# fateshelled/sycl_points

Measured on AMD Instinct MI355X. Metric: gicp_correspondences_per_sec, higher is better.
Workload: dtype f32

## Files before the change

sycl_points_amd/_lib.py:

```python
import ctypes as C
import os
import subprocess

_HERE = os.path.dirname(os.path.abspath(__file__))
LIB_PATH = os.environ.get("SP_AMD_LIB") or os.path.join(_HERE, "lib", "libsycl_points_amd.so")
CSRC = os.path.join(_HERE, "csrc")

SP_OK, SP_ERR_INVALID_ARGUMENT, SP_ERR_RUNTIME, SP_ERR_HIP = 0, 1, 2, 3
COMM_ID_BYTES = 128


class SpError(RuntimeError):

    def __init__(self, code, msg):
        super().__init__(f"[sycl_points_amd] error {code}: {msg}")
        self.code = code


class Linearized(C.Structure):
    _fields_ = [("H", C.c_float * 36), ("b", C.c_float * 6), ("error", C.c_float), ("inlier", C.c_uint32),
                ("inlier_lo", C.c_float), ("inlier_hi", C.c_float), ("pad", C.c_float * 2)]


class FactorParams(C.Structure):
# ... 356 lines not shown
    "sp_ogm_extract_visible_points": (_i, [_vp, _vp, _f, _f, _f, _vp, _vp, _vp, _vp, _vp, _sz, C.POINTER(_sz), _vp]),
    "sp_ogm_overlap_ratio": (_i, [_vp, _vp, _sz, _vp, C.POINTER(_f), _vp]),
    "sp_ogm_voxel_probability": (_i, [_vp, _vp, C.POINTER(_f), _vp]),
    "sp_ogm_export": (_i, [_vp, _vp, _vp, _vp, _vp, _vp, _vp, _vp, _vp, _vp, _sz, C.POINTER(_sz), _vp]),
    "sp_pc2_resolve_fields_host": (_i, [C.POINTER(C.c_char_p), C.POINTER(C.c_uint32), C.POINTER(C.c_uint8), _sz, C.c_uint32, _i, _i, _i,
                                        C.POINTER(Pc2Layout)]),
    "sp_pc2_unpack_workspace_bytes": (_sz, [_sz]),
    "sp_pc2_unpack": (_i, [_vp, _sz, _sz, C.POINTER(Pc2Layout), _vp, _vp, _vp, _vp, _vp, _vp, _vp]),
    "sp_pc2_pack_point_step": (C.c_uint32, [_i, _i, _i]),
    "sp_pc2_pack": (_i, [_vp, _vp, _vp, _vp, _sz, C.c_double, _vp, _vp]),
    "sp_enhanced_reflectivity_workspace_bytes": (_sz, [_sz]),
    "sp_enhanced_reflectivity": (_i, [_vp, _vp, _sz, _vp, C.c_uint32, C.c_int32, _i, C.c_int32, _vp, _f, _f, _vp, _vp]),
}


INTERNAL_SIGNATURES = {
    "sp_internal_source_option": (_i, [_vp, _i, _i]),
    "sp_internal_grid_option": (_i, [_vp, _i, _i]),
    "sp_internal_bvh_option": (_i, [_vp, _i, _i]),
    "sp_internal_grid_small_build": (_i, [_i]),
    "sp_internal_align_searched_log": (_vp, [_vp, _vp]),
    "sp_internal_source_tile_floats": (_sz, [_vp]),
    "sp_internal_source_tiles_copy": (_i, [_vp, _vp, _sz, _i, _vp]),
    "sp_internal_radix_sort_workspace_bytes": (_sz, [_sz]),
    "sp_internal_radix_sort_u32": (_i, [_vp, _vp, _vp, _vp, _sz, C.c_uint, _vp, _sz, _vp, _vp]),
    "sp_internal_radix_sort_u32_ex": (_i, [_vp, _vp, _vp, _vp, _sz, C.c_uint, C.c_uint, _i, _vp, _sz, _vp, _vp]),
    "sp_internal_radix_first_pass": (None, [_sz, C.c_uint, _vp]),
    "sp_internal_radix_sort_u64": (_i, [_vp, _vp, _vp, _vp, _sz, C.c_uint, _vp, _sz, _vp, _vp]),
    "sp_internal_exclusive_scan_workspace_bytes": (_sz, [_sz]),
    "sp_internal_exclusive_scan_u32": (_i, [_vp, _vp, _sz, _vp, _vp, _sz, _vp]),
    "sp_internal_atan2f_host": (None, [_vp, _vp, _sz, _vp]),
    "sp_internal_fps": (_i, [_i, _vp, _sz, _sz, C.c_uint32, _vp, _vp, _vp, _vp, _sz, _vp]),
    "sp_internal_eigen3": (_i, [_vp, _sz, _vp, _vp, _vp]),
    "sp_internal_inverse3": (_i, [_vp, _sz, _vp, _vp]),
    "sp_internal_bbox": (_i, [_vp, _sz, C.c_uint, _vp, _vp]),
    "sp_internal_morton_keys": (_i, [_vp, _sz, _vp, _vp, _i, _vp, _vp]),
    "sp_internal_sorted_insert": (_i, [_i, _i, _i, _vp, _vp, _sz, _sz, _vp, _vp, _vp]),
}
VOXEL_BOX_SHARDS, VOXEL_BOX_SHARD_STRIDE = 16, 32
COORD = {"LIDAR": 0, "CAMERA": 1}
FPS_FORM = {"auto": 0, "one_workgroup": 1, "per_sample": 2, "persistent": 3}
INTERNAL_OPTION = {"stage_mask": 0, "reuse": 1, "fast_nn": 2, "self_knn_mode": 3, "persistent": 4, "persistent_from": 5,
                   "bvh_self_heap": 6, "bvh_sort_queries": 7, "grid_sort_queries": 8, "opt_wave_query": 9, "opt_fuse_trials": 10}


def build(force=False):
    srcs = [os.path.join(CSRC, f) for f in os.listdir(CSRC) if f.endswith((".hip", ".h"))]
    srcs.append(os.path.join(_HERE, "..", "include", "sycl_points_amd.h"))
    stale = (not os.path.exists(LIB_PATH)) or any(os.path.getmtime(s) > os.path.getmtime(LIB_PATH) for s in srcs)
    if force or stale:
        subprocess.check_call(["make", "-C", CSRC, "-j8", "-s"])
    return LIB_PATH


_lib = None


def lib():
    global _lib
    if _lib is None:
        if not os.path.exists(LIB_PATH):
            raise ImportError(f"{LIB_PATH} is missing: run `python -c 'import __graft_entry__ as g; g.build()'` "
                              "(there is no CPU fallback for the HIP path)")
        import torch

        L = C.CDLL(LIB_PATH)
        for name, (res, args) in list(SIGNATURES.items()) + list(INTERNAL_SIGNATURES.items()):
            fn = getattr(L, name)
            fn.restype = res
            fn.argtypes = args
        if L.sp_abi_version() != 7:
            raise ImportError("libsycl_points_amd.so ABI version mismatch")
        _lib = L
    return _lib


def check(code):
    if code != SP_OK:
        raise SpError(code, lib().sp_last_error().decode())
```

sycl_points_amd/csrc/grid_device.h:

```cpp
#pragma once
#include "sp_common.h"
#include "sp_math.h"

struct sp_grid {
    size_t n = 0;
    float h = 1.0f, inv_h = 1.0f, eps = 0.0f;
    float org[3] = {0, 0, 0};
    int dims[3] = {1, 1, 1};
    size_t ncells = 1;
    float4* d_pts = nullptr;
    uint32_t* d_start = nullptr;
    mutable uint32_t* d_unit_off = nullptr;
    mutable uint32_t n_units = 0;
    mutable bool units_ready = false;
    hipStream_t build_stream = nullptr;
    hipEvent_t built_ev = nullptr;
    mutable uint32_t max_cell = 0;
    mutable bool max_cell_known = false;
    int self_knn_mode = 0;
    int sort_queries = 1;
    mutable sp::StreamSet streams;
};

namespace sp {

inline void grid_use(const sp_grid* g, hipStream_t st) {
    if (g->built_ev != nullptr && st != g->build_stream) (void)hipStreamWaitEvent(st, g->built_ev, 0);
    g->streams.note(st);
}

int grid_search_own_points(const sp_grid* grid, size_t k, int32_t* idx_out, float* d2_out, hipStream_t st, float bound2 = FLT_MAX);

struct GridDesc {
    float inv_h, h, eps;
    float ox, oy, oz;
    int nx, ny, nz;
    unsigned n;
};

inline GridDesc grid_desc(const sp_grid* gr) {
    return GridDesc{gr->inv_h, gr->h, gr->eps, gr->org[0], gr->org[1], gr->org[2], gr->dims[0], gr->dims[1],
                    gr->dims[2], (unsigned)gr->n};
}

__device__ __forceinline__ int cell_coord(float v, float o, float inv_h, int dim) {
    const float t = floorf((v - o) * inv_h);
    return (int)fminf(fmaxf(t, 0.0f), (float)(dim - 1));
}

__device__ __forceinline__ float gap2(float v, float lo, float hi, float eps) {
    const float g = fmaxf(fmaxf(lo - v, v - hi) - eps, 0.0f);
    return g * g;
}

__device__ __forceinline__ void load4_dist2(const float4* __restrict__ pts, unsigned i, unsigned e, float qx, float qy, float qz,
                                            float4 (&p)[4], float (&d)[4]) {
#pragma unroll
    for (int j = 0; j < 4; ++j) p[j] = pts[j ? min(i + j, e - 1) : i];
#pragma unroll
    for (int j = 0; j < 4; ++j) d[j] = dist2(qx, qy, qz, p[j].x, p[j].y, p[j].z);
}

template <class Bound, class Scan>
__device__ __forceinline__ void grid_ring_walk(const unsigned* __restrict__ start, const GridDesc& g, float qx, float qy,
                                               float qz, int r_start, bool proven_before, Bound&& bound2, Scan&& scan) {
// ... 36 lines not shown
                }
            }
        }
        if (covered(r)) break;
    }
}

struct Nearest {
    float d2;
    int idx;
    unsigned pos;
    float x, y, z;
};

__device__ __forceinline__ Nearest grid_nn1(const float4* __restrict__ pts, const unsigned* __restrict__ start,
                                            const GridDesc& g, float qx, float qy, float qz,
                                            const Nearest* seed = nullptr, int r_start = 0) {
    Nearest best;
    best.d2 = FLT_MAX; best.idx = -1; best.pos = 0; best.x = best.y = best.z = 0.0f;
    if (!(isfinite(qx) && isfinite(qy) && isfinite(qz)) || g.n == 0) return best;
    if (seed) best = *seed;
    const int cx = cell_coord(qx, g.ox, g.inv_h, g.nx), cy = cell_coord(qy, g.oy, g.inv_h, g.ny),
              cz = cell_coord(qz, g.oz, g.inv_h, g.nz);
    const int rmax = max(max(g.nx, g.ny), g.nz);
    auto consider = [&](const float4 p, unsigned pos) {
        const float d = dist2(qx, qy, qz, p.x, p.y, p.z);
        const int pi = __float_as_int(p.w);
        if (d < best.d2 || (d == best.d2 && pi < best.idx)) {
            best.d2 = d; best.idx = pi; best.pos = pos; best.x = p.x; best.y = p.y; best.z = p.z;
        }
    };
    for (int r = r_start; r <= rmax; ++r) {
        const int z0 = max(cz - r, 0), z1 = min(cz + r, g.nz - 1);
        const int y0 = max(cy - r, 0), y1 = min(cy + r, g.ny - 1);
        const int x0 = max(cx - r, 0), x1 = min(cx + r, g.nx - 1);
        for (int z = z0; z <= z1; ++z) {
            const float dz2 = gap2(qz, g.oz + z * g.h, g.oz + (z + 1) * g.h, g.eps);
            if (dz2 > best.d2) continue;
            for (int y = y0; y <= y1; ++y) {
                const float dyz2 = dz2 + gap2(qy, g.oy + y * g.h, g.oy + (y + 1) * g.h, g.eps);
                if (dyz2 > best.d2) continue;
                const bool shell_row = (r == 0) || (z == cz - r) || (z == cz + r) || (y == cy - r) || (y == cy + r);
                const unsigned row = ((unsigned)z * g.ny + y) * g.nx;
                const int nseg = shell_row ? 1 : 2;
                for (int sgi = 0; sgi < nseg; ++sgi) {
                    int xa, xb;
                    if (shell_row) { xa = x0; xb = x1; }
// ... 14 lines not shown
                    }
                }
            }
        }
        float cov = FLT_MAX;
        if (cx - r > 0) cov = fminf(cov, qx - (g.ox + (cx - r) * g.h));
        if (cx + r < g.nx - 1) cov = fminf(cov, (g.ox + (cx + r + 1) * g.h) - qx);
        if (cy - r > 0) cov = fminf(cov, qy - (g.oy + (cy - r) * g.h));
        if (cy + r < g.ny - 1) cov = fminf(cov, (g.oy + (cy + r + 1) * g.h) - qy);
        if (cz - r > 0) cov = fminf(cov, qz - (g.oz + (cz - r) * g.h));
        if (cz + r < g.nz - 1) cov = fminf(cov, (g.oz + (cz + r + 1) * g.h) - qz);
        if (cov == FLT_MAX) break;
        cov = fmaxf(cov - g.eps, 0.0f);
        if (best.d2 < cov * cov) break;
    }
    return best;
}

struct FastFlat {
    unsigned o0, o1, o2, o3;
    unsigned c1, c2, c3, total;
};

__device__ __forceinline__ void fast_extents(const unsigned* __restrict__ start, const GridDesc& g, float qx, float qy,
                                             float qz, unsigned (&s)[4], unsigned (&e)[4], float& cov_cells) {
    const float fx = (qx - g.ox) * g.inv_h, fy = (qy - g.oy) * g.inv_h, fz = (qz - g.oz) * g.inv_h;
    const float cxf = fminf(fmaxf(floorf(fx), 0.0f), (float)(g.nx - 1));
    const float cyf = fminf(fmaxf(floorf(fy), 0.0f), (float)(g.ny - 1));
    const float czf = fminf(fmaxf(floorf(fz), 0.0f), (float)(g.nz - 1));
    const float tx = fx - cxf, ty = fy - cyf, tz = fz - czf;
    const bool lx = tx < 0.5f, ly = ty < 0.5f, lz = tz < 0.5f;
    const int cx = (int)cxf, cy = (int)cyf, cz = (int)czf;
    const int xa = max(cx - (lx ? 1 : 0), 0), xb = min(cx + (lx ? 0 : 1), g.nx - 1);
    const int ya = max(cy - (ly ? 1 : 0), 0), yb = min(cy + (ly ? 0 : 1), g.ny - 1);
    const int za = max(cz - (lz ? 1 : 0), 0), zb = min(cz + (lz ? 0 : 1), g.nz - 1);
    cov_cells = fminf(fminf(lx ? 1.0f - tx : tx, ly ? 1.0f - ty : ty), lz ? 1.0f - tz : tz);
    const unsigned r00 = ((unsigned)za * g.ny + ya) * g.nx + xa;
    const unsigned dy = yb != ya ? (unsigned)g.nx : 0u, dz = zb != za ? (unsigned)g.ny * g.nx : 0u;
    const unsigned w = (unsigned)(xb - xa) + 1u;
    const unsigned r01 = r00 + dy, r10 = r00 + dz, r11 = r10 + dy;
    struct Three { unsigned a, b, c; };
    const Three v0 = *reinterpret_cast<const Three*>(start + r00), v1 = *reinterpret_cast<const Three*>(start + r01),
                v2 = *reinterpret_cast<const Three*>(start + r10), v3 = *reinterpret_cast<const Three*>(start + r11);
    const bool two = w == 2u;
    s[0] = v0.a; e[0] = two ? v0.c : v0.b;
    s[1] = v1.a; e[1] = two ? v1.c : v1.b;
    s[2] = v2.a; e[2] = two ? v2.c : v2.b;
    s[3] = v3.a; e[3] = two ? v3.c : v3.b;
    if (dy == 0u) { e[1] = s[1]; e[3] = s[3]; }
    if (dz == 0u) { e[2] = s[2]; e[3] = s[3]; }
}

__device__ __forceinline__ FastFlat fast_flatten(const unsigned (&s)[4], const unsigned (&e)[4], bool usable) {
    FastFlat f;
    const unsigned n0 = e[0] - s[0], n1 = e[1] - s[1], n2 = e[2] - s[2], n3 = e[3] - s[3];
    f.c1 = n0; f.c2 = n0 + n1; f.c3 = f.c2 + n2;
    f.o0 = s[0]; f.o1 = s[1] - f.c1; f.o2 = s[2] - f.c2; f.o3 = s[3] - f.c3;
    f.total = usable ? f.c3 + n3 : 0u;
    return f;
}
__device__ __forceinline__ unsigned fast_pos(const FastFlat& f, unsigned jj) {
    return jj + (jj < f.c1 ? f.o0 : (jj < f.c2 ? f.o1 : (jj < f.c3 ? f.o2 : f.o3)));
}

template <int B>
__device__ __forceinline__ void fast_load(const float4* __restrict__ pts, const FastFlat& f, unsigned base,
                                          float4 (&cand)[B]) {
#pragma unroll
    for (int j = 0; j < B; ++j) cand[j] = pts[fast_pos(f, min(base + j, f.total - 1))];
}
__device__ __forceinline__ unsigned long long nn_key(float d2, int idx) {
    return ((unsigned long long)__float_as_uint(d2) << 32) | (unsigned)idx;
}
template <int B>
__device__ __forceinline__ void fast_eval(const FastFlat& f, unsigned base, const float4 (&cand)[B], float qx, float qy,
                                          float qz, unsigned long long& best_key, unsigned& bj) {
#pragma unroll
    for (int j = 0; j < B; ++j) {
        const float d = dist2(qx, qy, qz, cand[j].x, cand[j].y, cand[j].z);
        unsigned long long key = nn_key(d, __float_as_int(cand[j].w));
        key = (base + j < f.total) ? key : ~0ull;
        const bool better = key < best_key;
        best_key = better ? key : best_key;
        bj = better ? base + j : bj;
    }
}

__device__ __forceinline__ bool grid_nn1_fast(const float4* __restrict__ pts, const unsigned* __restrict__ start,
                                              const GridDesc& g, float qx, float qy, float qz, Nearest& best,
                                              float bound2 = FLT_MAX, const Nearest* seed = nullptr) {
    best.d2 = bound2; best.idx = -1; best.pos = 0; best.x = best.y = best.z = 0.0f;
    const bool usable = isfinite(qx) && isfinite(qy) && isfinite(qz) && g.n != 0;
    if (!usable) return true;
    if (seed) best = *seed;
    unsigned s[4], e[4];
    float cov_cells;
    fast_extents(start, g, qx, qy, qz, s, e, cov_cells);
    const FastFlat f = fast_flatten(s, e, true);
    const unsigned long long none = nn_key(best.d2, best.idx);
    unsigned long long key = none;
    unsigned bj = 0;
#ifndef SP_FAST_B
#define SP_FAST_B 12
#endif
    for (unsigned base = 0; base < f.total; base += SP_FAST_B) {
        float4 cand[SP_FAST_B];
        fast_load<SP_FAST_B>(pts, f, base, cand);
        fast_eval<SP_FAST_B>(f, base, cand, qx, qy, qz, key, bj);
    }
    if (key != none) {
        best.pos = fast_pos(f, bj);
        const float4 w = pts[best.pos];
        best.x = w.x; best.y = w.y; best.z = w.z;
        best.idx = __float_as_int(w.w);
        best.d2 = __uint_as_float((unsigned)(key >> 32));
    }
    const float cov = fmaxf(cov_cells * g.h - g.eps, 0.0f);
    return best.d2 < cov * cov;
}

// ... 237 lines not shown
    second2 = ub;
    if (winner != kNone && runner_up != kNone) second2 = fminf(ub, __uint_as_float((unsigned)(runner_up >> 32)));
    if (m < key_in) {
        const int wl = __ffsll((long long)__ballot(k1 == m)) - 1;
        const unsigned wpos = (unsigned)__builtin_amdgcn_readlane((int)bpos, wl);
        const float4 w = pts[wpos];
        best.d2 = __uint_as_float((unsigned)(m >> 32));
        best.idx = __float_as_int(w.w);
        best.pos = wpos;
        best.x = w.x; best.y = w.y; best.z = w.z;
    }
}

__device__ __forceinline__ void grid_nn1_later_stages(const float4* __restrict__ pts, const unsigned* __restrict__ start,
                                                      const GridDesc& g, float qx, float qy, float qz, Nearest& best) {
    if (grid_nn1_block4(pts, start, g, qx, qy, qz, best)) return;
    if (best.d2 < FLT_MAX && grid_nn1_ball(pts, start, g, qx, qy, qz, best)) return;
    const Nearest seed = best;
    best = grid_nn1(pts, start, g, qx, qy, qz, &seed, 2);
}

__device__ __forceinline__ Nearest grid_nn1_auto(const float4* __restrict__ pts, const unsigned* __restrict__ start,
                                                 const GridDesc& g, float qx, float qy, float qz, float bound2 = FLT_MAX,
                                                 const Nearest* seed = nullptr) {
    Nearest best;
    if (!grid_nn1_fast(pts, start, g, qx, qy, qz, best, bound2, seed)) grid_nn1_later_stages(pts, start, g, qx, qy, qz, best);
    return best;
}

}
```

sycl_points_amd/csrc/registration.hip:

```cpp
#include <algorithm>
#include <mutex>

#include "registration_device.h"
#include "sp_cov_normal.h"

namespace sp {
namespace {


struct PointTerm {
    float H[6][6];
    float b[6];
    float sq;
    float residual_norm;
    float genz_weight;
};

__device__ __forceinline__ void se3_jacobian(const Rigid& T, float px, float py, float pz, float J[3][6]) {
#pragma unroll
    for (int i = 0; i < 3; ++i) {
        const float r0 = T.R[i][0], r1 = T.R[i][1], r2 = T.R[i][2];
        J[i][0] = chain3(r0, 0.0f, r1, pz, r2, -py);
        J[i][1] = chain3(r0, -pz, r1, 0.0f, r2, px);
        J[i][2] = chain3(r0, py, r1, -px, r2, 0.0f);
// ... 636 lines not shown
            after_loads();
            if (threadIdx.x < kFanRow) red[1][threadIdx.x] = rv;
        }
        __syncthreads();
        if (threadIdx.x < kAcc - 1) red[0][threadIdx.x] = red[1][threadIdx.x];
        else if (threadIdx.x == kAcc - 1)
            red[0][kAcc - 1] = __uint_as_float((unsigned)red[1][kAcc] * 4096u + (unsigned)red[1][kAcc - 1]);
        else if (threadIdx.x == kAcc) red[0][kAcc] = red[1][kAcc + 1];
        __syncthreads();
        return true;
    }
}
__device__ __forceinline__ void align_store_late_state(const AlignArgs& A) {
    if (threadIdx.x < kStateWords) {
        unsigned w = A.has_prev ? reinterpret_cast<const unsigned*>(A.state_in)[threadIdx.x] : 0u;
        if (!A.has_prev && threadIdx.x < 16) w = __float_as_uint(A.T_init[threadIdx.x]);
        if (threadIdx.x == kStateFlagWord) w = 1u;
        if (threadIdx.x == kStateFlagWord + 3) w = 1u;
        reinterpret_cast<unsigned*>(A.state_out)[threadIdx.x] = w;
    }
}

template <bool SHARDED>
__device__ __forceinline__ bool align_prologue(const AlignArgs& A, float* sT, unsigned* sflag) {
    __shared__ float red[kFinalThreads / 32][kPartial];
    __shared__ sp_linearized slin;
    __shared__ float sdelta[8];
    __shared__ LdltScratch ldlt_ws;
    if (A.first) {
        state_store(state_load(false, nullptr, A.T_init), sT, sflag);
        if (!SHARDED && blockIdx.x == 0 && A.searched_log && threadIdx.x >= 64 && threadIdx.x < 64 + kSearchedLog)
            A.searched_log[threadIdx.x - 64] = 0u;
        __syncthreads();
        return true;
    }
    const unsigned sv = state_load(A.has_prev, A.state_in, A.T_init);
    const unsigned nrows = (SHARDED && A.mode == ALIGN_ROWS) ? (unsigned)kAlignMaxBlocks : gridDim.x;
    const bool arrived = align_totals<SHARDED>(A, A.prev_rows, nrows, red, [=] { state_store(sv, sT, sflag); }, sflag);
    if (!arrived) {
        if (blockIdx.x == 0) align_store_late_state(A);
        return false;
    }
    auto zero_row = [&] {
        if (SHARDED && A.mode == ALIGN_FANIN && blockIdx.x == 0 && threadIdx.x >= 64 && threadIdx.x < 64 + kFanRow)
            A.fan_row_out[threadIdx.x - 64] = 0.0f;
    };
    if (sflag[0]) {
        if (blockIdx.x == 0 && threadIdx.x < kStateWords)
            reinterpret_cast<unsigned*>(A.state_out)[threadIdx.x] = reinterpret_cast<const unsigned*>(A.state_in)[threadIdx.x];
        zero_row();
        return false;
    }
    if (threadIdx.x == 0)
        finish_iteration(red[0], sT, A.lambda, A.crit_rot, A.crit_trans, sflag[1], &slin, sdelta, &ldlt_ws, blockIdx.x == 0, A.state_out,
                         A.searched_log,
                         A.k, A.lin_out);
    __syncthreads();
    if (sdelta[6] > 0.5f) {
        zero_row();
        return false;
    }
    return true;
}

template <int LOSS, bool FAST_NN, bool P2D = false, bool SHARDED = false>
__global__ __launch_bounds__(kAlignBlock) void gicp_align_kernel(FusedParams P, AlignArgs A,
                                                                 float* __restrict__ partials) {
    __shared__ float sT[16];
    __shared__ unsigned sflag[2];
    if (!align_prologue<SHARDED>(A, sT, sflag)) return;
    const Rigid T = uniform_pose(sT);
    float acc[kAcc - 1];
    unsigned cnt = 0, searched = 0;
    const unsigned stride = gridDim.x * kAlignBlock;
#pragma unroll
    for (int e = 0; e < kAcc - 1; ++e) acc[e] = 0.0f;
    const unsigned tile = xcd_tile();
    for (unsigned i = tile * kAlignBlock + threadIdx.x; i < P.n; i += stride)
        fused_point<LOSS, FAST_NN, P2D, kSeedSearches, kNegCert>(P, T, i, acc, cnt, searched);
    if constexpr (!SHARDED) {
        block_reduce_store<kAcc - 1, kAlignBlock>(acc, cnt, partials + (size_t)blockIdx.x * kPartial, false, searched);
    } else if (A.mode == ALIGN_ROWS) {
        block_reduce_store<kAcc - 1, kAlignBlock>(acc, cnt, partials + (size_t)blockIdx.x * kPartial, true, searched);
    } else {
        block_reduce_store<kAcc - 1, kAlignBlock, true>(acc, cnt, partials + (size_t)blockIdx.x * kPartial, false, searched);
        align_tail(A, partials);
    }
}

struct PersistArgs {
    AlignWs ws;
    unsigned* tickets;
    const float* T_init;
    float lambda, crit_rot, crit_trans;
    sp_linearized* lin_out;
    float* T_out;
    float* delta_out8;
    uint32_t* iterations_out;
    int max_iterations;
    int k_begin;
    int cache_valid_later;
    unsigned long long budget;
// ... 899 lines not shown
    return SP_OK;
}

extern "C" int sp_gicp_source_set_wave_per_point(sp_gicp_source* s, int mode) {
    if (!s || mode < 0 || mode > 2) return SP_ERR_INVALID_ARGUMENT;
    s->opt_wave_query = mode;
    return SP_OK;
}

extern "C" const uint32_t* sp_internal_align_searched_log(void* workspace, size_t* n_entries_out) {
    if (n_entries_out) *n_entries_out = sp::kSearchedLog;
    return workspace ? sp::align_ws(workspace).searched_log : nullptr;
}
extern "C" size_t sp_internal_source_tile_floats(const sp_gicp_source* s) {
    return s ? sp::src_tile_words(s->n_max ? s->n_max : 1) : 0;
}
extern "C" int sp_internal_source_tiles_copy(sp_gicp_source* s, float* device_buffer, size_t n_floats, int to_source, void* stream) {
    if (!s || !device_buffer || n_floats != sp_internal_source_tile_floats(s)) return SP_ERR_INVALID_ARGUMENT;
    const hipError_t e = hipMemcpyAsync(to_source ? s->tiles : device_buffer, to_source ? device_buffer : s->tiles,
                                        n_floats * sizeof(float), hipMemcpyDeviceToDevice, sp::as_stream(stream));
    if (e != hipSuccess) { sp_set_error(hipGetErrorString(e)); return SP_ERR_HIP; }
    return SP_OK;
}
extern "C" int sp_internal_source_option(sp_gicp_source* s, int option, int value) {
    if (!s) return SP_ERR_INVALID_ARGUMENT;
    switch (option) {
        case SP_INTERNAL_FUSED_STAGE_MASK: s->opt_stage_mask = value; return SP_OK;
        case SP_INTERNAL_FUSED_REUSE: s->opt_reuse = value; s->cache_valid = false; return SP_OK;
        case SP_INTERNAL_FUSED_FAST_NN: s->opt_fast_nn = value; return SP_OK;
        case SP_INTERNAL_FUSED_PERSISTENT: s->opt_persistent = value; return SP_OK;
        case SP_INTERNAL_FUSED_PERSISTENT_FROM: s->opt_persistent_from = value < 0 ? 0 : value; return SP_OK;
        case SP_INTERNAL_OPT_WAVE_QUERY: s->opt_wave_query = value; return SP_OK;
        case SP_INTERNAL_OPT_FUSE_TRIALS: s->opt_fuse_trials = value; return SP_OK;
    }
    return SP_ERR_INVALID_ARGUMENT;
}
```

sycl_points_amd/csrc/registration_device.h:

```cpp
#ifndef SP_REGISTRATION_DEVICE_H
#define SP_REGISTRATION_DEVICE_H

#include "grid_device.h"
#include "radix_sort.h"
#include "sp_linearize.h"
#include "sp_xchg.h"

#include <type_traits>

void sp_set_error(const char* msg);

#include "sp_internal.h"

namespace sp {
namespace {

constexpr int kAcc = 29;
constexpr int kPartial = 32;
constexpr int kMaxBlocks = 1024;

template <bool SC1>
__device__ __forceinline__ void store_row_word(float* p, float v) {
    if (SC1) __hip_atomic_store(p, v, __ATOMIC_RELAXED, __HIP_MEMORY_SCOPE_AGENT);
    else *p = v;
// ... 180 lines not shown
__device__ __forceinline__ Sym3 load_sym(const float4* __restrict__ p) {
    const float4 a = p[0], b = p[1];
    return Sym3{a.x, a.y, a.z, a.w, b.x, b.y};
}

constexpr unsigned kSrcPlanes = 9;
constexpr unsigned kSrcTileWords = kSrcPlanes * kWave;
__host__ __device__ inline size_t src_tile_words(size_t n) { return (n + kWave - 1) / kWave * kSrcTileWords; }

struct FusedParams {
    const float* src;
    const float4* tpts;
    const unsigned* tstart;
    const float4* tcovp;
    const float4* tnb;
    GridDesc g;
    unsigned n;
    float max_d2, scale;
    Mat4Arg T_val;
    const float* T_dev;
    const unsigned* perm;
    float4* ccache;
    int cache_valid;
    int32_t* nn_idx;
    float* nn_d2;
};

__device__ __forceinline__ const float* src_words(const FusedParams& P, unsigned i) {
    return P.src + ((size_t)(i / kWave) * kSrcTileWords + (i % kWave));
}
__device__ __forceinline__ float4 src_point(const float* __restrict__ w) {
    return make_float4(w[0], w[kWave], w[2 * kWave], 1.0f);
}
__device__ __forceinline__ Sym3 src_cov(const float* __restrict__ w) {
    return Sym3{w[3 * kWave], w[4 * kWave], w[5 * kWave], w[6 * kWave], w[7 * kWave], w[8 * kWave]};
}

template <int LOSS, bool P2D = false, bool ERR_ONLY = false, int NACC = kAcc - 1>
__device__ __forceinline__ void fused_math(const FusedParams& P, const Rigid& T, const float4 s, float qx, float qy,
                                           float qz, const Nearest& nn, const Sym3& Cs, const Sym3& Ct,
                                           float (&acc)[NACC], unsigned& cnt) {
    float t[NACC];
    linearize_terms<LOSS, P2D, ERR_ONLY>(T, s.x, s.y, s.z, qx, qy, qz, nn.x, nn.y, nn.z, Cs, Ct, P.scale, t);
#pragma unroll
    for (int e = 0; e < NACC; ++e) acc[e] += t[e];
    ++cnt;
}

__device__ __forceinline__ void store_correspondence(float4* __restrict__ row, const FusedParams& P, const Nearest& nn,
                                                     Sym3& Ct, float qx = 0.0f, float qy = 0.0f, float qz = 0.0f,
                                                     float margin2 = 0.0f) {
    float4 r0 = make_float4(qx, qy, qz, margin2), r1 = make_float4(0.0f, 0.0f, 0.0f, 0.0f),
           r2 = make_float4(0.0f, 0.0f, __int_as_float(-1), 0.0f);
    if (nn.idx >= 0) {
        const float4 c0 = P.tcovp[2 * (size_t)nn.pos], c1 = P.tcovp[2 * (size_t)nn.pos + 1];
        r0 = make_float4(nn.x, nn.y, nn.z, c1.z);
        r1 = c0;
        r2 = make_float4(c1.x, c1.y, __int_as_float(nn.idx), __uint_as_float(nn.pos));
        Ct = Sym3{c0.x, c0.y, c0.z, c0.w, c1.x, c1.y};
    }
    row[0] = r0;
    row[1] = r1;
    row[2] = r2;
}

__device__ __forceinline__ bool certified(const FusedParams& P, float d, float rho2, float qx, float qy, float qz,
                                          unsigned pos) {
    if (d < rho2) return true;
    if (!P.tnb || !(rho2 > 0.0f)) return false;
    const float4 nb = P.tnb[pos];
    return d < nb.w && d < dist2(qx, qy, qz, nb.x, nb.y, nb.z);
}

__device__ __forceinline__ float search_bound2(const FusedParams& P) {
    return (P.nn_idx == nullptr && P.max_d2 < FLT_MAX) ? __uint_as_float(__float_as_uint(P.max_d2) + 1u) : FLT_MAX;
}
__device__ __forceinline__ float search_bound2_margin(const FusedParams& P, float& margin2) {
    margin2 = 0.0f;
    if (P.nn_idx != nullptr || !(P.max_d2 < FLT_MAX) || P.ccache == nullptr) return search_bound2(P);
    const float B = sqrtf(P.max_d2), m = 0.25f * B;
    const float wide = (B + m) * (B + m);
    if (!(wide < FLT_MAX)) return search_bound2(P);
    margin2 = (0.98f * m) * (0.98f * m);
    return wide;
}

template <int LOSS, bool FAST_NN, bool P2D = false, bool SEED = true, bool NEG = true>
__device__ __forceinline__ void fused_point(const FusedParams& P, const Rigid& T, unsigned i, float (&acc)[kAcc - 1],
                                            unsigned& cnt, unsigned& searched) {
    const float* const sw = src_words(P, i);
    const float4 s = src_point(sw);
    float4* const row = P.ccache + 3 * (size_t)i;
    float qx, qy, qz;
    transform_point(T, s.x, s.y, s.z, qx, qy, qz);
    Nearest nn;
    Sym3 Ct{0.0f, 0.0f, 0.0f, 0.0f, 0.0f, 0.0f};
    bool hit = false;
    bool seeded = false;
    Nearest seed;
    seed.d2 = FLT_MAX; seed.idx = -1; seed.pos = 0; seed.x = seed.y = seed.z = 0.0f;
    if (P.cache_valid) {
        const float4 r0 = row[0], r1 = row[1], r2 = row[2];
        const float d = dist2(qx, qy, qz, r0.x, r0.y, r0.z);
        const unsigned pos = __float_as_uint(r2.w);
        if (certified(P, d, r0.w, qx, qy, qz, pos)) {
            hit = true;
            nn.idx = __float_as_int(r2.z); nn.pos = pos; nn.x = r0.x; nn.y = r0.y; nn.z = r0.z;
            nn.d2 = nn.idx >= 0 ? d : FLT_MAX;
            Ct = Sym3{r1.x, r1.y, r1.z, r1.w, r2.x, r2.y};
        } else if (SEED && __float_as_int(r2.z) >= 0) {
            seed.d2 = d; seed.idx = __float_as_int(r2.z); seed.pos = pos; seed.x = r0.x; seed.y = r0.y; seed.z = r0.z;
            seeded = true;
        }
    }
    if (!hit) {
        ++searched;
        float margin2 = 0.0f;
        const float bound2 = NEG ? search_bound2_margin(P, margin2) : search_bound2(P);
        seeded = seeded && seed.d2 < bound2;
        if (!seeded) { seed.d2 = bound2; seed.idx = -1; seed.pos = 0; seed.x = seed.y = seed.z = 0.0f; }
        if (FAST_NN) {
            nn = grid_nn1_auto(P.tpts, P.tstart, P.g, qx, qy, qz, bound2, &seed);
        } else {
            nn = grid_nn1(P.tpts, P.tstart, P.g, qx, qy, qz, &seed, 0);
        }
        if (NEG) store_correspondence(row, P, nn, Ct, qx, qy, qz, margin2);
        else store_correspondence(row, P, nn, Ct);
    }
    if (P.nn_idx) {
        const unsigned o = P.perm[i];
        P.nn_idx[o] = nn.idx;
        P.nn_d2[o] = nn.d2;
    }
    if (nn.idx < 0 || nn.d2 > P.max_d2) return;
    unsigned i_again = i;
    asm volatile("" : "+v"(i_again));
    const float* const sw_again = src_words(P, i_again);
    const Sym3 Cs = P2D ? Sym3{0.0f, 0.0f, 0.0f, 0.0f, 0.0f, 0.0f} : src_cov(sw_again);
    fused_math<LOSS, P2D>(P, T, src_point(sw_again), qx, qy, qz, nn, Cs, Ct, acc, cnt);
}

#ifdef SP_OPT_TIMING
__device__ unsigned long long g_sp_dbg[24 * 16];
__device__ unsigned g_sp_step;
__device__ unsigned long long g_sp_wg[24 * 8];
#define SP_PSTAMP(k) if (blockIdx.x == 0 && threadIdx.x == 0 && g_sp_step < 24) g_sp_dbg[g_sp_step * 16 + (k)] = wall_clock64()
#else
#define SP_PSTAMP(k)
#endif
template <int LOSS, bool P2D = false>
__device__ __forceinline__ void fused_point_wave(const FusedParams& P, const Rigid& T, unsigned i, bool valid,
                                                 float (&acc)[kAcc - 1], unsigned& cnt, unsigned& searched) {
    const unsigned ii = valid ? i : 0u;
    SP_PSTAMP(0);
    const float* const sw = src_words(P, ii);
    const float4 s = src_point(sw);
    float qx, qy, qz;
    transform_point(T, s.x, s.y, s.z, qx, qy, qz);
    Nearest nn;
    nn.d2 = FLT_MAX; nn.idx = -1; nn.pos = 0; nn.x = nn.y = nn.z = 0.0f;
    Sym3 Ct{0.0f, 0.0f, 0.0f, 0.0f, 0.0f, 0.0f};
    bool hit = false;
// ... 254 lines not shown
    void note(hipStream_t st) const { streams.note(st); if (grid) sp::grid_use(grid, st); }
};
namespace sp {
constexpr size_t kOptRowsBytes = 2 * (size_t)256 * 32 * sizeof(unsigned long long);
}
struct sp_gicp_source {
    size_t n_max = 0, n = 0;
    float* tiles = nullptr;
    unsigned* perm = nullptr;
    float4* ccache = nullptr;
    float4* qcert = nullptr;
    float4* qcert2 = nullptr;
    size_t qcert_points = 0;
    mutable bool qcert_valid = false;
    float4* ccache2 = nullptr;
    unsigned long long* opt_rows = nullptr;
    mutable unsigned opt_epoch = 0;
    mutable bool cache_valid = false;
    const sp_gicp_target* cache_target = nullptr;
    unsigned long long cache_version = 0;
    bool sorted = false;
    int opt_stage_mask = 3;
    int opt_reuse = 2;
    int opt_fast_nn = -1;
    int opt_persistent = 1;
    int opt_persistent_from = 4;
    int opt_fuse_trials = 1;
    int opt_wave_query = 1;
    unsigned *keys_in = nullptr, *keys_out = nullptr, *vals_in = nullptr;
    void* sort_tmp = nullptr;
    size_t sort_tmp_bytes = 0;
};

namespace sp {
namespace {
FusedParams make_fused_params(const sp_gicp_target* target, const sp_gicp_source* source, const sp_factor_params* params,
                              const float* transT, int transT_on_device, int32_t* nn_idx_out, float* nn_d2_out) {
    const size_t n = source->n;
    FusedParams P;
    P.src = source->tiles;
    P.tpts = target->grid->d_pts;
    P.tstart = target->grid->d_start;
    P.tcovp = target->covp;
    P.tnb = source->opt_reuse > 1 ? target->nb : nullptr;
    P.g = grid_desc(target->grid);
    P.n = (unsigned)n;
    P.max_d2 = params->max_correspondence_distance * params->max_correspondence_distance;
    P.scale = params->robust_scale;
    for (int i = 0; i < 16; ++i) P.T_val.m[i] = (i % 5 == 0) ? 1.0f : 0.0f;
    if (transT && !transT_on_device)
        for (int i = 0; i < 16; ++i) P.T_val.m[i] = transT[i];
    P.T_dev = transT_on_device ? transT : nullptr;
    P.perm = source->perm;
    P.ccache = source->ccache;
    P.cache_valid = (source->opt_reuse && source->cache_valid && source->cache_target == target &&
                     source->cache_version == target->version) ? 1 : 0;
    P.nn_idx = (nn_idx_out && nn_d2_out) ? nn_idx_out : nullptr;
    P.nn_d2 = nn_d2_out;
    return P;
}

int check_prepared_reg(const sp_gicp_target* target, const sp_factor_params* params) {
    if (params->reg_type != SP_REG_GICP && params->reg_type != SP_REG_POINT_TO_DISTRIBUTION) {
        sp_set_error("[sp_gicp_*] only RegType::GICP and RegType::POINT_TO_DISTRIBUTION have a prepared/fused form");
        return SP_ERR_INVALID_ARGUMENT;
    }
    if (params->reg_type != target->reg_type) {
        sp_set_error("[sp_gicp_*] the prepared target holds the rows of another RegType: call sp_gicp_target_prepare");
        return SP_ERR_INVALID_ARGUMENT;
    }
    if (params->rotation_constraint_enable) {
        sp_set_error("[sp_gicp_*] the rotation constraint needs the raw covariances: use sp_gicp_linearize");
        return SP_ERR_INVALID_ARGUMENT;
    }
    return SP_OK;
}

int check_workspace(const void* workspace, size_t workspace_bytes, size_t n) {
    if (!workspace || workspace_bytes < sp_gicp_workspace_bytes(n)) {
// ... 77 lines not shown
```

sycl_points_amd/csrc/sp_internal.h:

```cpp
#ifndef SP_INTERNAL_H
#define SP_INTERNAL_H

#include "../../include/sycl_points_amd.h"

#ifdef __cplusplus
extern "C" {
#endif

enum {
    SP_INTERNAL_FUSED_STAGE_MASK = 0,
    SP_INTERNAL_FUSED_REUSE = 1,
    SP_INTERNAL_FUSED_FAST_NN = 2,
    SP_INTERNAL_SELF_KNN_MODE = 3,
    SP_INTERNAL_FUSED_PERSISTENT = 4,
    SP_INTERNAL_FUSED_PERSISTENT_FROM = 5,
    SP_INTERNAL_BVH_SELF_HEAP = 6,
    SP_INTERNAL_BVH_SORT_QUERIES = 7,
    SP_INTERNAL_GRID_SORT_QUERIES = 8,
    SP_INTERNAL_OPT_WAVE_QUERY = 9,
    SP_INTERNAL_OPT_FUSE_TRIALS = 10
};

int sp_internal_source_option(sp_gicp_source* source, int option, int value);
int sp_internal_grid_option(sp_grid* grid, int option, int value);
int sp_internal_bvh_option(sp_bvh* bvh, int option, int value);
int sp_internal_grid_small_build(int enable);
const uint32_t* sp_internal_align_searched_log(void* workspace, size_t* n_entries_out);
size_t sp_internal_source_tile_floats(const sp_gicp_source* source);
int sp_internal_source_tiles_copy(sp_gicp_source* source, float* device_buffer, size_t n_floats, int to_source, void* stream);
size_t sp_internal_radix_sort_workspace_bytes(size_t n);
int sp_internal_radix_sort_u32(uint32_t* keys_a, uint32_t* keys_b, uint32_t* vals_a, uint32_t* vals_b, size_t n,
                               unsigned bits, void* workspace, size_t workspace_bytes, int* result_in_b_out, void* stream);
int sp_internal_radix_sort_u32_ex(uint32_t* keys_a, uint32_t* keys_b, uint32_t* vals_a, uint32_t* vals_b, size_t n,
                                  unsigned bits, unsigned first_bit, int first_hist_ready, void* workspace,
                                  size_t workspace_bytes, int* result_in_b_out, void* stream);
void sp_internal_radix_first_pass(size_t n, unsigned bits, unsigned* out4);
int sp_internal_radix_sort_u64(uint64_t* keys_a, uint64_t* keys_b, uint32_t* vals_a, uint32_t* vals_b, size_t n,
                               unsigned bits, void* workspace, size_t workspace_bytes, int* result_in_b_out, void* stream);
size_t sp_internal_exclusive_scan_workspace_bytes(size_t n);
int sp_internal_exclusive_scan_u32(const uint32_t* in, uint32_t* out, size_t n, uint32_t* total_out_or_null, void* workspace,
                                   size_t workspace_bytes, void* stream);
void sp_internal_atan2f_host(const float* y, const float* x, size_t n, float* out);
int sp_internal_fps(int form, const float* points, size_t n, size_t sampling_num, uint32_t first_index, uint32_t* order_out,
                    uint8_t* flags_out_opt, float* min_d2_out_opt, void* workspace, size_t workspace_bytes, void* stream);
int sp_internal_eigen3(const float* covs, size_t n, float* vals_out, float* vecs_out, void* stream);
int sp_internal_inverse3(const float* mats, size_t n, float* out, void* stream);
int sp_internal_bbox(const float* points, size_t n, unsigned workgroups, uint32_t* box6_words_out, void* stream);
int sp_internal_morton_keys(const float* points, size_t n, const float* lo3, const float* hi3, int mode, uint64_t* keys_out,
                            void* stream);
int sp_internal_sorted_insert(int order, int kcap, int k, const float* d, const int32_t* idx, size_t rows, size_t m, float* d_out,
                              int32_t* idx_out, void* stream);

// ... 5 lines not shown
```

Baseline: 31.99 billion.

## Add adaptive searching launch mode that prefetches grid extents before cache check

Adds a search mode for the fused GICP align kernel. When the previous iteration searched more than half the points, it launches a variant that issues the grid-cell extent loads before the cache check, so memory latency overlaps. That variant also replaces certification with a plain radius test. It also adds a bound check before loading neighbour certification data, scalar-register hints for grid dims, and a cache-row copy debug entry. The costs are extra register pressure and a second kernel code path.

```diff
diff --git a/sycl_points_amd/_lib.py b/sycl_points_amd/_lib.py
--- a/sycl_points_amd/_lib.py
+++ b/sycl_points_amd/_lib.py
@@ -402,6 +402,7 @@
     "sp_internal_align_searched_log": (_vp, [_vp, _vp]),
     "sp_internal_source_tile_floats": (_sz, [_vp]),
     "sp_internal_source_tiles_copy": (_i, [_vp, _vp, _sz, _i, _vp]),
+    "sp_internal_source_cache_rows_copy": (_i, [_vp, _vp, _sz, _vp]),
     "sp_internal_radix_sort_workspace_bytes": (_sz, [_sz]),
     "sp_internal_radix_sort_u32": (_i, [_vp, _vp, _vp, _vp, _sz, C.c_uint, _vp, _sz, _vp, _vp]),
     "sp_internal_radix_sort_u32_ex": (_i, [_vp, _vp, _vp, _vp, _sz, C.c_uint, C.c_uint, _i, _vp, _sz, _vp, _vp]),
@@ -421,7 +422,7 @@
 COORD = {"LIDAR": 0, "CAMERA": 1}
 FPS_FORM = {"auto": 0, "one_workgroup": 1, "per_sample": 2, "persistent": 3}
 INTERNAL_OPTION = {"stage_mask": 0, "reuse": 1, "fast_nn": 2, "self_knn_mode": 3, "persistent": 4, "persistent_from": 5,
-                   "bvh_self_heap": 6, "bvh_sort_queries": 7, "grid_sort_queries": 8, "opt_wave_query": 9, "opt_fuse_trials": 10}
+                   "bvh_self_heap": 6, "bvh_sort_queries": 7, "grid_sort_queries": 8, "opt_wave_query": 9, "opt_fuse_trials": 10, "search_mode": 11}
 
 
 def build(force=False):
@@ -446,6 +447,8 @@
 
         L = C.CDLL(LIB_PATH)
         for name, (res, args) in list(SIGNATURES.items()) + list(INTERNAL_SIGNATURES.items()):
+            if name in INTERNAL_SIGNATURES and os.environ.get("SP_AMD_LIB") and not hasattr(L, name):
+                continue
             fn = getattr(L, name)
             fn.restype = res
             fn.argtypes = args
diff --git a/sycl_points_amd/csrc/grid_device.h b/sycl_points_amd/csrc/grid_device.h
--- a/sycl_points_amd/csrc/grid_device.h
+++ b/sycl_points_amd/csrc/grid_device.h
@@ -41,6 +41,11 @@
 inline GridDesc grid_desc(const sp_grid* gr) {
     return GridDesc{gr->inv_h, gr->h, gr->eps, gr->org[0], gr->org[1], gr->org[2], gr->dims[0], gr->dims[1],
                     gr->dims[2], (unsigned)gr->n};
+}
+
+__device__ __forceinline__ int here(int uniform_value) {
+    asm volatile("" : "+s"(uniform_value));
+    return uniform_value;
 }
 
 __device__ __forceinline__ int cell_coord(float v, float o, float inv_h, int dim) {
@@ -123,7 +128,7 @@
     if (seed) best = *seed;
     const int cx = cell_coord(qx, g.ox, g.inv_h, g.nx), cy = cell_coord(qy, g.oy, g.inv_h, g.ny),
               cz = cell_coord(qz, g.oz, g.inv_h, g.nz);
-    const int rmax = max(max(g.nx, g.ny), g.nz);
+    const int rmax = max(max(here(g.nx), g.ny), g.nz);
     auto consider = [&](const float4 p, unsigned pos) {
         const float d = dist2(qx, qy, qz, p.x, p.y, p.z);
         const int pi = __float_as_int(p.w);
@@ -184,12 +189,17 @@
     unsigned c1, c2, c3, total;
 };
 
-__device__ __forceinline__ void fast_extents(const unsigned* __restrict__ start, const GridDesc& g, float qx, float qy,
-                                             float qz, unsigned (&s)[4], unsigned (&e)[4], float& cov_cells) {
+struct FastRequest {
+    struct Three { unsigned a, b, c; };
+    Three v0, v1, v2, v3;
+    bool two, no_y, no_z;
+};
+__device__ __forceinline__ FastRequest fast_extents_request(const unsigned* __restrict__ start, const GridDesc& g, float qx,
+                                                            float qy, float qz, float& cov_cells) {
     const float fx = (qx - g.ox) * g.inv_h, fy = (qy - g.oy) * g.inv_h, fz = (qz - g.oz) * g.inv_h;
-    const float cxf = fminf(fmaxf(floorf(fx), 0.0f), (float)(g.nx - 1));
-    const float cyf = fminf(fmaxf(floorf(fy), 0.0f), (float)(g.ny - 1));
-    const float czf = fminf(fmaxf(floorf(fz), 0.0f), (float)(g.nz - 1));
+    const float cxf = fminf(fmaxf(floorf(fx), 0.0f), (float)here(g.nx - 1));
+    const float cyf = fminf(fmaxf(floorf(fy), 0.0f), (float)here(g.ny - 1));
+    const float czf = fminf(fmaxf(floorf(fz), 0.0f), (float)here(g.nz - 1));
     const float tx = fx - cxf, ty = fy - cyf, tz = fz - czf;
     const bool lx = tx < 0.5f, ly = ty < 0.5f, lz = tz < 0.5f;
     const int cx = (int)cxf, cy = (int)cyf, cz = (int)czf;
@@ -201,16 +211,28 @@
     const unsigned dy = yb != ya ? (unsigned)g.nx : 0u, dz = zb != za ? (unsigned)g.ny * g.nx : 0u;
     const unsigned w = (unsigned)(xb - xa) + 1u;
     const unsigned r01 = r00 + dy, r10 = r00 + dz, r11 = r10 + dy;
-    struct Three { unsigned a, b, c; };
-    const Three v0 = *reinterpret_cast<const Three*>(start + r00), v1 = *reinterpret_cast<const Three*>(start + r01),
-                v2 = *reinterpret_cast<const Three*>(start + r10), v3 = *reinterpret_cast<const Three*>(start + r11);
-    const bool two = w == 2u;
-    s[0] = v0.a; e[0] = two ? v0.c : v0.b;
-    s[1] = v1.a; e[1] = two ? v1.c : v1.b;
-    s[2] = v2.a; e[2] = two ? v2.c : v2.b;
-    s[3] = v3.a; e[3] = two ? v3.c : v3.b;
-    if (dy == 0u) { e[1] = s[1]; e[3] = s[3]; }
-    if (dz == 0u) { e[2] = s[2]; e[3] = s[3]; }
+    using Three = FastRequest::Three;
+    FastRequest f;
+    f.v0 = *reinterpret_cast<const Three*>(start + r00);
+    f.v1 = *reinterpret_cast<const Three*>(start + r01);
+    f.v2 = *reinterpret_cast<const Three*>(start + r10);
+    f.v3 = *reinterpret_cast<const Three*>(start + r11);
+    f.two = w == 2u;
+    f.no_y = dy == 0u;
+    f.no_z = dz == 0u;
+    return f;
+}
+__device__ __forceinline__ void fast_extents_ranges(const FastRequest& f, unsigned (&s)[4], unsigned (&e)[4]) {
+    s[0] = f.v0.a; e[0] = f.two ? f.v0.c : f.v0.b;
+    s[1] = f.v1.a; e[1] = f.two ? f.v1.c : f.v1.b;
+    s[2] = f.v2.a; e[2] = f.two ? f.v2.c : f.v2.b;
+    s[3] = f.v3.a; e[3] = f.two ? f.v3.c : f.v3.b;
+    if (f.no_y) { e[1] = s[1]; e[3] = s[3]; }
+    if (f.no_z) { e[2] = s[2]; e[3] = s[3]; }
+}
+__device__ __forceinline__ void fast_extents(const unsigned* __restrict__ start, const GridDesc& g, float qx, float qy,
+                                             float qz, unsigned (&s)[4], unsigned (&e)[4], float& cov_cells) {
+    fast_extents_ranges(fast_extents_request(start, g, qx, qy, qz, cov_cells), s, e);
 }
 
 __device__ __forceinline__ FastFlat fast_flatten(const unsigned (&s)[4], const unsigned (&e)[4], bool usable) {
@@ -250,14 +272,16 @@
 
 __device__ __forceinline__ bool grid_nn1_fast(const float4* __restrict__ pts, const unsigned* __restrict__ start,
                                               const GridDesc& g, float qx, float qy, float qz, Nearest& best,
-                                              float bound2 = FLT_MAX, const Nearest* seed = nullptr) {
+                                              float bound2 = FLT_MAX, const Nearest* seed = nullptr,
+                                              const FastRequest* requested = nullptr, float requested_cov_cells = 0.0f) {
     best.d2 = bound2; best.idx = -1; best.pos = 0; best.x = best.y = best.z = 0.0f;
     const bool usable = isfinite(qx) && isfinite(qy) && isfinite(qz) && g.n != 0;
     if (!usable) return true;
     if (seed) best = *seed;
     unsigned s[4], e[4];
-    float cov_cells;
-    fast_extents(start, g, qx, qy, qz, s, e, cov_cells);
+    float cov_cells = requested_cov_cells;
+    if (requested) fast_extents_ranges(*requested, s, e);
+    else fast_extents(start, g, qx, qy, qz, s, e, cov_cells);
     const FastFlat f = fast_flatten(s, e, true);
     const unsigned long long none = nn_key(best.d2, best.idx);
     unsigned long long key = none;
@@ -541,9 +565,11 @@
 
 __device__ __forceinline__ Nearest grid_nn1_auto(const float4* __restrict__ pts, const unsigned* __restrict__ start,
                                                  const GridDesc& g, float qx, float qy, float qz, float bound2 = FLT_MAX,
-                                                 const Nearest* seed = nullptr) {
+                                                 const Nearest* seed = nullptr, const FastRequest* requested = nullptr,
+                                                 float requested_cov_cells = 0.0f) {
     Nearest best;
-    if (!grid_nn1_fast(pts, start, g, qx, qy, qz, best, bound2, seed)) grid_nn1_later_stages(pts, start, g, qx, qy, qz, best);
+    if (!grid_nn1_fast(pts, start, g, qx, qy, qz, best, bound2, seed, requested, requested_cov_cells))
+        grid_nn1_later_stages(pts, start, g, qx, qy, qz, best);
     return best;
 }
 
diff --git a/sycl_points_amd/csrc/registration.hip b/sycl_points_amd/csrc/registration.hip
--- a/sycl_points_amd/csrc/registration.hip
+++ b/sycl_points_amd/csrc/registration.hip
@@ -682,12 +682,13 @@
 }
 
 template <bool SHARDED>
-__device__ __forceinline__ bool align_prologue(const AlignArgs& A, float* sT, unsigned* sflag) {
+__device__ __forceinline__ bool align_prologue(const AlignArgs& A, float* sT, unsigned* sflag, unsigned* searched_prev = nullptr) {
     __shared__ float red[kFinalThreads / 32][kPartial];
     __shared__ sp_linearized slin;
     __shared__ float sdelta[8];
     __shared__ LdltScratch ldlt_ws;
     if (A.first) {
+        if (searched_prev && threadIdx.x == 0) *searched_prev = 0u;
         state_store(state_load(false, nullptr, A.T_init), sT, sflag);
         if (!SHARDED && blockIdx.x == 0 && A.searched_log && threadIdx.x >= 64 && threadIdx.x < 64 + kSearchedLog)
             A.searched_log[threadIdx.x - 64] = 0u;
@@ -711,10 +712,12 @@
         zero_row();
         return false;
     }
-    if (threadIdx.x == 0)
+    if (threadIdx.x == 0) {
+        if (searched_prev) *searched_prev = (unsigned)red[0][kAcc];
         finish_iteration(red[0], sT, A.lambda, A.crit_rot, A.crit_trans, sflag[1], &slin, sdelta, &ldlt_ws, blockIdx.x == 0, A.state_out,
                          A.searched_log,
                          A.k, A.lin_out);
+    }
     __syncthreads();
     if (sdelta[6] > 0.5f) {
         zero_row();
@@ -728,7 +731,8 @@
                                                                  float* __restrict__ partials) {
     __shared__ float sT[16];
     __shared__ unsigned sflag[2];
-    if (!align_prologue<SHARDED>(A, sT, sflag)) return;
+    __shared__ unsigned searched_prev;
+    if (!align_prologue<SHARDED>(A, sT, sflag, &searched_prev)) return;
     const Rigid T = uniform_pose(sT);
     float acc[kAcc - 1];
     unsigned cnt = 0, searched = 0;
@@ -736,8 +740,16 @@
 #pragma unroll
     for (int e = 0; e < kAcc - 1; ++e) acc[e] = 0.0f;
     const unsigned tile = xcd_tile();
-    for (unsigned i = tile * kAlignBlock + threadIdx.x; i < P.n; i += stride)
-        fused_point<LOSS, FAST_NN, P2D, kSeedSearches, kNegCert>(P, T, i, acc, cnt, searched);
+    bool searching = false;
+    if constexpr (!SHARDED && FAST_NN) searching = searching_launch(P, searched_prev);
+    if (searching) {
+        if constexpr (!SHARDED && FAST_NN)
+            for (unsigned i = tile * kAlignBlock + threadIdx.x; i < P.n; i += stride)
+                fused_point<LOSS, FAST_NN, P2D, kSeedSearches, kNegCert, true>(P, T, i, acc, cnt, searched);
+    } else {
+        for (unsigned i = tile * kAlignBlock + threadIdx.x; i < P.n; i += stride)
+            fused_point<LOSS, FAST_NN, P2D, kSeedSearches, kNegCert>(P, T, i, acc, cnt, searched);
+    }
     if constexpr (!SHARDED) {
         block_reduce_store<kAcc - 1, kAlignBlock>(acc, cnt, partials + (size_t)blockIdx.x * kPartial, false, searched);
     } else if (A.mode == ALIGN_ROWS) {
@@ -1683,6 +1695,13 @@
     if (e != hipSuccess) { sp_set_error(hipGetErrorString(e)); return SP_ERR_HIP; }
     return SP_OK;
 }
+extern "C" int sp_internal_source_cache_rows_copy(const sp_gicp_source* s, float* device_buffer, size_t n_floats, void* stream) {
+    if (!s || !device_buffer || !s->ccache || n_floats != 12 * s->n) return SP_ERR_INVALID_ARGUMENT;
+    if (n_floats == 0) return SP_OK;
+    const hipError_t e = hipMemcpyAsync(device_buffer, s->ccache, n_floats * sizeof(float), hipMemcpyDeviceToDevice, sp::as_stream(stream));
+    if (e != hipSuccess) { sp_set_error(hipGetErrorString(e)); return SP_ERR_HIP; }
+    return SP_OK;
+}
 extern "C" int sp_internal_source_option(sp_gicp_source* s, int option, int value) {
     if (!s) return SP_ERR_INVALID_ARGUMENT;
     switch (option) {
@@ -1693,6 +1712,10 @@
         case SP_INTERNAL_FUSED_PERSISTENT_FROM: s->opt_persistent_from = value < 0 ? 0 : value; return SP_OK;
         case SP_INTERNAL_OPT_WAVE_QUERY: s->opt_wave_query = value; return SP_OK;
         case SP_INTERNAL_OPT_FUSE_TRIALS: s->opt_fuse_trials = value; return SP_OK;
+        case SP_INTERNAL_FUSED_SEARCH_MODE:
+            if (value < 0 || value > 2) return SP_ERR_INVALID_ARGUMENT;
+            s->opt_search_mode = value;
+            return SP_OK;
     }
     return SP_ERR_INVALID_ARGUMENT;
 }
diff --git a/sycl_points_amd/csrc/registration_device.h b/sycl_points_amd/csrc/registration_device.h
--- a/sycl_points_amd/csrc/registration_device.h
+++ b/sycl_points_amd/csrc/registration_device.h
@@ -226,6 +226,7 @@
     const unsigned* perm;
     float4* ccache;
     int cache_valid;
+    int search_mode;
     int32_t* nn_idx;
     float* nn_d2;
 };
@@ -269,10 +270,11 @@
 }
 
 __device__ __forceinline__ bool certified(const FusedParams& P, float d, float rho2, float qx, float qy, float qz,
-                                          unsigned pos) {
+                                          unsigned pos, float bound2 = FLT_MAX) {
     if (d < rho2) return true;
-    if (!P.tnb || !(rho2 > 0.0f)) return false;
-    const float4 nb = P.tnb[pos];
+    if (!P.tnb || !(rho2 > 0.0f) || !(d < bound2)) return false;
+    float4 nb = P.tnb[pos];
+    asm volatile("" : "+v"(nb.x), "+v"(nb.y), "+v"(nb.z), "+v"(nb.w));
     return d < nb.w && d < dist2(qx, qy, qz, nb.x, nb.y, nb.z);
 }
 
@@ -289,9 +291,10 @@
     return wide;
 }
 
-template <int LOSS, bool FAST_NN, bool P2D = false, bool SEED = true, bool NEG = true>
+template <int LOSS, bool FAST_NN, bool P2D = false, bool SEED = true, bool NEG = true, bool SEARCHING = false>
 __device__ __forceinline__ void fused_point(const FusedParams& P, const Rigid& T, unsigned i, float (&acc)[kAcc - 1],
                                             unsigned& cnt, unsigned& searched) {
+    static_assert(!SEARCHING || FAST_NN, "the searching form requests the extents of the fast path");
     const float* const sw = src_words(P, i);
     const float4 s = src_point(sw);
     float4* const row = P.ccache + 3 * (size_t)i;
@@ -303,11 +306,14 @@
     bool seeded = false;
     Nearest seed;
     seed.d2 = FLT_MAX; seed.idx = -1; seed.pos = 0; seed.x = seed.y = seed.z = 0.0f;
-    if (P.cache_valid) {
+    FastRequest requested;
+    float requested_cov_cells = 0.0f;
+    if (SEARCHING || P.cache_valid) {
+        if (SEARCHING) requested = fast_extents_request(P.tstart, P.g, qx, qy, qz, requested_cov_cells);
         const float4 r0 = row[0], r1 = row[1], r2 = row[2];
         const float d = dist2(qx, qy, qz, r0.x, r0.y, r0.z);
         const unsigned pos = __float_as_uint(r2.w);
-        if (certified(P, d, r0.w, qx, qy, qz, pos)) {
+        if (SEARCHING ? d < r0.w : certified(P, d, r0.w, qx, qy, qz, pos, NEG ? FLT_MAX : search_bound2(P))) {
             hit = true;
             nn.idx = __float_as_int(r2.z); nn.pos = pos; nn.x = r0.x; nn.y = r0.y; nn.z = r0.z;
             nn.d2 = nn.idx >= 0 ? d : FLT_MAX;
@@ -324,7 +330,7 @@
         seeded = seeded && seed.d2 < bound2;
         if (!seeded) { seed.d2 = bound2; seed.idx = -1; seed.pos = 0; seed.x = seed.y = seed.z = 0.0f; }
         if (FAST_NN) {
-            nn = grid_nn1_auto(P.tpts, P.tstart, P.g, qx, qy, qz, bound2, &seed);
+                        nn = grid_nn1_auto(P.tpts, P.tstart, P.g, qx, qy, qz, bound2, &seed, SEARCHING ? &requested : nullptr, requested_cov_cells);
         } else {
             nn = grid_nn1(P.tpts, P.tstart, P.g, qx, qy, qz, &seed, 0);
         }
@@ -342,6 +348,14 @@
     const float* const sw_again = src_words(P, i_again);
     const Sym3 Cs = P2D ? Sym3{0.0f, 0.0f, 0.0f, 0.0f, 0.0f, 0.0f} : src_cov(sw_again);
     fused_math<LOSS, P2D>(P, T, src_point(sw_again), qx, qy, qz, nn, Cs, Ct, acc, cnt);
+}
+
+#ifndef SP_SEARCH_MODE_EIGHTHS
+#define SP_SEARCH_MODE_EIGHTHS 4
+#endif
+__device__ __forceinline__ bool searching_launch(const FusedParams& P, unsigned searched_prev) {
+    if (!P.cache_valid || P.g.n == 0 || P.search_mode == 0) return false;
+    return P.search_mode == 2 || searched_prev > (unsigned)(((unsigned long long)P.n * SP_SEARCH_MODE_EIGHTHS) >> 3);
 }
 
 #ifdef SP_OPT_TIMING
@@ -642,6 +656,7 @@
     bool sorted = false;
     int opt_stage_mask = 3;
     int opt_reuse = 2;
+    int opt_search_mode = 1;
     int opt_fast_nn = -1;
     int opt_persistent = 1;
     int opt_persistent_from = 4;
@@ -675,6 +690,7 @@
     P.ccache = source->ccache;
     P.cache_valid = (source->opt_reuse && source->cache_valid && source->cache_target == target &&
                      source->cache_version == target->version) ? 1 : 0;
+    P.search_mode = source->opt_search_mode;
     P.nn_idx = (nn_idx_out && nn_d2_out) ? nn_idx_out : nullptr;
     P.nn_d2 = nn_d2_out;
     return P;
diff --git a/sycl_points_amd/csrc/sp_internal.h b/sycl_points_amd/csrc/sp_internal.h
--- a/sycl_points_amd/csrc/sp_internal.h
+++ b/sycl_points_amd/csrc/sp_internal.h
@@ -18,7 +18,8 @@
     SP_INTERNAL_BVH_SORT_QUERIES = 7,
     SP_INTERNAL_GRID_SORT_QUERIES = 8,
     SP_INTERNAL_OPT_WAVE_QUERY = 9,
-    SP_INTERNAL_OPT_FUSE_TRIALS = 10
+    SP_INTERNAL_OPT_FUSE_TRIALS = 10,
+    SP_INTERNAL_FUSED_SEARCH_MODE = 11
 };
 
 int sp_internal_source_option(sp_gicp_source* source, int option, int value);
@@ -28,6 +29,7 @@
 const uint32_t* sp_internal_align_searched_log(void* workspace, size_t* n_entries_out);
 size_t sp_internal_source_tile_floats(const sp_gicp_source* source);
 int sp_internal_source_tiles_copy(sp_gicp_source* source, float* device_buffer, size_t n_floats, int to_source, void* stream);
+int sp_internal_source_cache_rows_copy(const sp_gicp_source* source, float* device_buffer, size_t n_floats, void* stream);
 size_t sp_internal_radix_sort_workspace_bytes(size_t n);
 int sp_internal_radix_sort_u32(uint32_t* keys_a, uint32_t* keys_b, uint32_t* vals_a, uint32_t* vals_b, size_t n,
                                unsigned bits, void* workspace, size_t workspace_bytes, int* result_in_b_out, void* stream);
```

After: 32.24 billion (median of 5 runs). No clear change (+0.8%).
